# AutomationLabs-sh/AutomationLabsModelPredictiveControl.jl

Measured on AMD Instinct MI355X. Metric: MPC steps/s (batch=4096, nx=12, nu=4, N=30), higher is better.
Workload: dtype f64; 1 GPU; configs[1]: hover-linearised quadrotor nx=12 nu=4 N=30, 4096 instances per GPU, shared model, x0 amplitude classes 0.3/1.0/3.0 interleaved, cold start every step; batch_per_gpu=4096, global_batch=4096, seed=0x5eed0002, setup_ramp_steps=300, admm_max_iter=6, check_every=6, polish=1, warm_state_kept=False, parallelism=instances sharded over 1 GPU(s), 16-instance tile per workgroup

## Files before the change

automationlabsmodelpredictivecontrol.jl_amd/_capi.py:

```python
from __future__ import annotations

import ctypes
import os

import numpy as np

_HERE = os.path.dirname(os.path.abspath(__file__))
LIB_PATH = os.environ.get("ALMPC_LIB") or os.path.join(_HERE, "lib", "libalmpc.so")

ALMPC_OK = 0
ERR_NAMES = {0: "ALMPC_OK", -1: "ALMPC_ERR_INVALID", -2: "ALMPC_ERR_NO_DEVICE", -3: "ALMPC_ERR_HIP",
             -4: "ALMPC_ERR_UNSUPPORTED", -5: "ALMPC_ERR_NOT_DESIGNED", -6: "ALMPC_ERR_NUMERIC"}
FLAG_TIMING = 0x1
FLAG_STRUCTURED = 0x2
SOLVED, MAX_ITER, NON_FINITE, INFEASIBLE = 0, 1, 2, 3


class AlmpcError(RuntimeError):
    def __init__(self, code, msg=""):
        self.code = code
        super().__init__(f"{ERR_NAMES.get(code, code)}: {msg}")


class almpc_opts(ctypes.Structure):
# ... 144 lines not shown
    L.almpc_group_sqp_fnn_skipped.argtypes = [_hp, _ip]
    L.almpc_group_sqp_fnn_state_multipliers.argtypes = [_hp, _dp]
    L.almpc_group_sqp_fnn_solve.argtypes = [_hp, ctypes.c_int, ctypes.c_double, ctypes.POINTER(almpc_opts), _ip, _ip, _dp]
    L.almpc_group_x0_staging.argtypes = [_hp, ctypes.POINTER(_dp)]
    L.almpc_group_update_initialization_staged.argtypes = [_hp, ctypes.POINTER(_dp)]
    L.almpc_group_get_results_async.argtypes = [_hp, ctypes.c_uint32]
    L.almpc_group_get_results_wait.argtypes = [_hp, ctypes.c_int, _dp, _dp, _dp, _dp, _dp, _ip, _ip, _ip]
    for nm_ in ("almpc_group_set_terminal_equality", "almpc_group_set_rho_profile", "almpc_group_set_structured_fallback", "almpc_group_set_state_box",
                "almpc_group_design_batched", "almpc_group_relin_fnn_setup", "almpc_group_relin_fnn_step", "almpc_group_relin_fnn_step_async",
                "almpc_group_relin_fnn_advance", "almpc_group_advance_plant", "almpc_group_sqp_fnn_set_structured", "almpc_group_sqp_fnn_set_step_rule",
                "almpc_group_sqp_fnn_setup", "almpc_group_relin_densenet_setup", "almpc_group_sqp_densenet_setup", "almpc_group_sqp_fnn_start", "almpc_group_sqp_fnn_iterate", "almpc_group_sqp_fnn_skipped", "almpc_group_sqp_fnn_solve", "almpc_group_sqp_fnn_set_hessian",
                "almpc_group_sqp_fnn_set_row_multipliers", "almpc_group_sqp_fnn_state_multipliers",
                "almpc_group_x0_staging", "almpc_group_update_initialization_staged", "almpc_group_get_results_async", "almpc_group_get_results_wait"):
        getattr(L, nm_).restype = ctypes.c_int
    L.almpc_set_start_from.argtypes = [_hp, _hp]
    L.almpc_set_start_from.restype = ctypes.c_int
    L.almpc_timing_samples.argtypes = [_hp, ctypes.c_int, ctypes.POINTER(ctypes.c_int), _fp, _fp, _fp, _fp]
    L.almpc_timing_samples.restype = ctypes.c_int
    for name in ("almpc_x0_staging", "almpc_update_initialization_async", "almpc_get_results_async", "almpc_get_results_wait", "almpc_host_results",
                 "almpc_get_first_input", "almpc_group_create", "almpc_group_size", "almpc_group_shard", "almpc_group_design_shared",
                 "almpc_group_set_reference", "almpc_group_update_initialization", "almpc_group_calculate",
                 "almpc_group_calculate_async", "almpc_group_synchronize", "almpc_group_get_results"):
        getattr(L, name).restype = ctypes.c_int
    for name in ("almpc_create", "almpc_design_shared", "almpc_set_reference", "almpc_update_initialization",
                 "almpc_update_initialization_device", "almpc_calculate", "almpc_calculate_async", "almpc_synchronize",
                 "almpc_get_results", "almpc_get_design", "almpc_device_results", "almpc_get_timing", "almpc_timing_reset",
                 "almpc_timing_summary"):
        getattr(L, name).restype = ctypes.c_int
    _lib = L
    return L


OPT_NO_WARM_STATE = 0x1
WANT = {"x": 0x01, "e_x": 0x02, "u": 0x04, "e_u": 0x08, "status": 0x10, "iters": 0x20, "polish_iters": 0x40, "u0": 0x80}


def _want_mask(want):
    try:
        return sum(WANT[k] for k in set(want))
    except KeyError as e:
        raise ValueError(f"unknown result {e.args[0]!r}; choose from {sorted(WANT)}") from None


def comm_unique_id() -> bytes:
    buf = ctypes.create_string_buffer(128)
    rc = load().almpc_comm_unique_id(buf)
    if rc != ALMPC_OK:
        raise AlmpcError(rc, "almpc_comm_unique_id (librccl not loadable?)")
    return buf.raw


def default_opts(**kw) -> almpc_opts:
    o = almpc_opts()
    load().almpc_default_opts(ctypes.byref(o))
    if "keep_warm_state" in kw:
        if not kw.pop("keep_warm_state"):
            o.reserved[0] |= OPT_NO_WARM_STATE
    for k, v in kw.items():
        if not hasattr(o, k):
            raise TypeError(f"unknown solver option {k!r}")
        setattr(o, k, v)
    return o


def _colmajor(a, shape=None):
    a = np.asfortranarray(np.asarray(a, dtype=np.float64))
    if shape is not None and a.shape != shape:
        raise ValueError(f"expected shape {shape}, got {a.shape}")
    return a


def _ptr(a):
    return None if a is None else a.ctypes.data_as(_dp)


def dare(A, B, Q, R):
    L = load()
    A, B = np.asfortranarray(A, dtype=np.float64), np.asfortranarray(B, dtype=np.float64)
    n, m = B.shape
    Q, R = _colmajor(Q, (n, n)), _colmajor(R, (m, m))
    P = np.empty((n, n), order="F")
    rc = L.almpc_dare(n, m, _ptr(A), _ptr(B), _ptr(Q), _ptr(R), _ptr(P))
    if rc != ALMPC_OK:
        raise AlmpcError(rc, "almpc_dare")
    return P


FNN_ACTIVATIONS = {"identity": 0, "relu": 1, "tanh": 2, "sigmoid": 3, "swish": 4}
NET_KINDS = {"fnn", "resnet", "polynet"}
_NET_CODES = {"fnn": 0, "resnet": 1, "polynet": 2}
# ... 727 lines not shown
```

automationlabsmodelpredictivecontrol.jl_amd/csrc/almpc_api.hip:

```cpp
#include "almpc_kernels.hip.h"
#include "almpc_design.hip.h"
#include "almpc_polish_gen.hip.h"
#include "almpc_fnn.hip.h"
#include "almpc_instance.hip.h"
#include "almpc_sqp.hip.h"
#include "almpc_comm.hip.h"
#include "almpc_riccati.hip.h"
#include "almpc_sdual.hip.h"
#include "almpc_host_math.h"
#include "almpc_switches.h"
#include "../../include/almpc.h"

#ifndef ALMPC_UNITY
#define ALMPC_KERNEL_INSTANCE(...) extern template __global__ __VA_ARGS__;
#include "instances/sdual_a.inc"
#include "instances/sdual_b.inc"
#include "instances/sdual_c.inc"
#include "instances/polish_gen.inc"
#include "instances/step.inc"
#include "instances/instance.inc"
#include "instances/design_a.inc"
#include "instances/design_b.inc"
#undef ALMPC_KERNEL_INSTANCE
#endif
// ... 1948 lines not shown
    per_wave = (per_wave + 1) & ~1;
    if (h->batched) {
        L.wave_const_off = per_wave;
        per_wave += (h->nzs + h->n * (h->n + h->m) + 1) & ~1;
    }
    L.per_wave = per_wave;
    L.SL = polish_shared_layout(h->n, h->m, h->N, h->nz, h->nzs, L.fuse_rollout);
    L.g_lds = (size_t)h->nz * ((h->nz + 1) & ~1);
    L.l_glds = (L.g_lds + L.SL.total + (size_t)POLISH_WAVES_GLDS * per_wave + 2) * sizeof(double);
    const size_t slot = (size_t)POLISH_SG_SHARED_CAP * 64 * sizeof(double);
    if (L.l_glds + slot <= 160 * 1024 && !h->batched && !h->sw.polish_sg_global) {
        L.sg_shared_off = (int)(L.SL.total + (size_t)POLISH_WAVES_GLDS * per_wave + 2);
        L.l_glds += slot;
    }
    L.l_step = L.l_glds - L.g_lds * sizeof(double);
    if (admm_lds_bytes(h) > L.l_step) L.l_step = admm_lds_bytes(h);
    L.l_step += L.g_lds * sizeof(double);
    return L;
}

PolishParams polish_params(const Step& s, const PolishLayout& L) {
    const almpc_handle* h = s.h;
    PolishParams pp;
    pp.nz = h->nz; pp.m = h->m; pp.batch = h->batch; pp.nzs = h->nzs;
    pp.G = h->batched ? h->bG : h->dG; pp.dvec = h->batched ? h->bD : h->dD;
    pp.G_stride = h->batched ? (long)h->nz * h->nzs : 0; pp.d_stride = h->batched ? (long)h->nzs : 0;
    pp.A_stride = h->batched ? (long)h->n * h->n : 0; pp.B_stride = h->batched ? (long)h->n * h->m : 0;
    pp.wave_const_off = L.wave_const_off; pp.sg_off = 0; pp.g_off = 0; pp.sg_shared_off = L.sg_shared_off;
    pp.umin = h->dUmin; pp.umax = h->dUmax; pp.uref = h->dUref; pp.uref_stride = h->uref_stride;
    pp.zs = h->dZs; pp.ys = h->dYs; pp.v0 = h->dV0; pp.w = h->dW; pp.status = h->dStatus; pp.piters = h->dPiters;
    pp.yflags = s.keep_state ? nullptr : h->dYflags; pp.yflag_words = h->nrb;
    pp.sglobal = h->dSglobal; pp.perm = h->dPerm; pp.ntiles = (h->batch + 15) / 16;
    pp.max_iter = s.o.polish_max_iter > 0 ? s.o.polish_max_iter : 2 * h->nz + 50;
    pp.dflag = s.mode.fold_flag ? h->bFlag : nullptr;
    if (s.lazy_redo) { pp.unsolved = h->redo.dUnsolved; pp.redo_gate = h->redo.dGate; pp.step_serial = h->redo.step_serial; }
    pp.fuse_rollout = L.fuse_rollout; pp.roll_g = s.roll.g; pp.roll_cpl = s.roll.cpl; pp.roll = s.rp;
    pp.rollM = h->dRollM; pp.roll_s = h->roll_s; pp.roll_nb = h->roll_nb;
    pp.lds_per_wave = L.per_wave;
    return pp;
}

enum class Route { StateRows, FusedShared, WaveShared, WaveInst, TwoLaunch, NoPolish };

Route pick_route(const Step& s, const PolishLayout& L) {
    const almpc_handle* h = s.h;
    if (h->mc > 0) return Route::StateRows;
    if (!s.o.polish) return Route::NoPolish;
    if (!h->batched && h->fuse_step && POLISH_WAVES_GLDS == 8 && !h->sw.polish_no_glds && h->nrb == 8 && (h->ks == 30 || h->ks == 32) && L.fused &&
        L.l_step <= 160 * 1024)
        return Route::FusedShared;
    if (!h->batched && h->nzs <= 64 && L.fused && h->dPlain && !h->ltv && !h->sw.no_shared_wave &&
        (long)h->batch <= h->sw.shared_wave_max_batch.value_or((long)2 * h->num_cus) && ((size_t)L.SL.total + (size_t)L.per_wave) * sizeof(double) <= 64 * 1024)
        return Route::WaveShared;
    if (h->batched && s.mode.guess == Guess::Admm && h->nzs <= 64 && L.fused && !h->sw.no_inst_wave &&
        ((size_t)L.SL.total + (size_t)L.per_wave + (size_t)h->nz * h->nzs) * sizeof(double) <= 64 * 1024)
        return Route::WaveInst;
    return Route::TwoLaunch;
}

template <bool PACKED>
hipError_t launch_admm_inst(const AdmmInstParams& ip, int wgs, size_t lds, hipStream_t st) {
    if (lds > 64 * 1024) {
        const hipError_t e = ensure_dyn_lds(reinterpret_cast<const void*>(k_admm_inst<PACKED>), lds);
        if (e != hipSuccess) return e;
    }
    hipLaunchKernelGGL((k_admm_inst<PACKED>), dim3(wgs), dim3(ADMM_INST_THREADS), lds, st, ip);
// ... 1588 lines not shown
```

automationlabsmodelpredictivecontrol.jl_amd/csrc/almpc_kernels.hip.h:

```cpp
#pragma once
#include <hip/hip_runtime.h>
#include <stdint.h>

#include <map>
#include <mutex>
#include <utility>
#include <type_traits>

namespace almpc {

inline hipError_t ensure_dyn_lds(const void* fn, size_t bytes) {
    if (bytes <= 64 * 1024) return hipSuccess;
    static std::mutex mu;
    static std::map<std::pair<int, const void*>, size_t> cur;
    int dev = 0;
    hipError_t e = hipGetDevice(&dev);
    if (e != hipSuccess) return e;
    std::lock_guard<std::mutex> lock(mu);
    size_t& c = cur[std::make_pair(dev, fn)];
    if (c >= bytes) return hipSuccess;
    e = hipFuncSetAttribute(fn, hipFuncAttributeMaxDynamicSharedMemorySize, (int)bytes);
    if (e == hipSuccess) c = bytes;
    return e;
}


#ifdef ALMPC_STAMPS
__device__ long long* g_stamps = nullptr;
#define ALMPC_STAMP(WAVE_ID, SLOT)                                                                     \
    do {                                                                                               \
        __builtin_amdgcn_sched_barrier(0);                                                             \
        if (g_stamps && (threadIdx.x & 63) == 0) g_stamps[(size_t)(WAVE_ID) * 16 + (SLOT)] = __builtin_readcyclecounter(); \
        __builtin_amdgcn_sched_barrier(0);                                                             \
    } while (0)
#define ALMPC_ACC_DECL long long acc_t[8] = {0, 0, 0, 0, 0, 0, 0, 0}; long long acc_prev = 0; int acc_n = 0;
#define ALMPC_ACC_START do { __builtin_amdgcn_sched_barrier(0); acc_prev = __builtin_readcyclecounter(); __builtin_amdgcn_sched_barrier(0); } while (0)
#define ALMPC_ACC(SLOT) do { __builtin_amdgcn_sched_barrier(0); const long long n_ = __builtin_readcyclecounter(); acc_t[SLOT] += n_ - acc_prev; acc_prev = n_; __builtin_amdgcn_sched_barrier(0); } while (0)
#define ALMPC_ACC_FLUSH(WAVE_ID) do { if (g_stamps && (threadIdx.x & 63) == 0) { for (int i_ = 0; i_ < 8; ++i_) g_stamps[(size_t)(4096 + (WAVE_ID)) * 16 + i_] = acc_t[i_]; g_stamps[(size_t)(4096 + (WAVE_ID)) * 16 + 8] = acc_n; } } while (0)
#else
#define ALMPC_STAMP(WAVE_ID, SLOT) do { } while (0)
#define ALMPC_ACC_DECL
#define ALMPC_ACC_START do { } while (0)
#define ALMPC_ACC(SLOT) do { } while (0)
#define ALMPC_ACC_FLUSH(WAVE_ID) do { } while (0)
#endif

__host__ __device__ inline int packed_tri_off(int nz, int c) {
    const int full = c * nz - (c * (c - 1)) / 2;
    const int pads = (nz & 1) ? (c / 2) : ((c + 1) / 2);
    return full + pads;
}
__host__ __device__ inline long packed_tri_doubles(int nz) { return ((long)packed_tri_off(nz, nz) + 1) & ~1L; }

typedef double d4 __attribute__((ext_vector_type(4)));
typedef double d2v __attribute__((ext_vector_type(2)));

constexpr int TILE = 16;

__device__ __forceinline__ d4 mfma_f64(double a, double b, d4 c) {
    return __builtin_amdgcn_mfma_f64_16x16x4f64(a, b, c, 0, 0, 0);
}

template <int KS>
__device__ __forceinline__ d4 tile_matmul(const double (&a)[KS], const double* bbuf, int q, int col) {
    d4 acc0 = {0.0, 0.0, 0.0, 0.0}, acc1 = {0.0, 0.0, 0.0, 0.0};
#pragma unroll
    for (int ks = 0; ks < KS; ks += 2) {
        double b0 = bbuf[(4 * ks + q) * TILE + col];
        acc0 = mfma_f64(a[ks], b0, acc0);
        if (ks + 1 < KS) {
            double b1 = bbuf[(4 * (ks + 1) + q) * TILE + col];
// ... 212 lines not shown
        if (check) {
            double rp = 0, nx = 0, nzn = 0, rd = 0, nhx = 0, ny = 0, bad = 0;
            for (int w2 = 0; w2 < NRB; ++w2) {
                const double* r = red + w2 * 8 * TILE + col;
                rp = fmax(rp, r[0 * TILE]); nx = fmax(nx, r[1 * TILE]); nzn = fmax(nzn, r[2 * TILE]);
                rd = fmax(rd, r[3 * TILE]); nhx = fmax(nhx, r[4 * TILE]); ny = fmax(ny, r[5 * TILE]);
                bad = fmax(bad, r[6 * TILE]);
            }
            if (active) {
                const bool conv = (rp <= p.eps_abs + p.eps_rel * fmax(nx, nzn)) &&
                                  (rd <= p.eps_abs + p.eps_rel * fmax(fmax(nhx, ny), nf));
                if (bad > 0.0) { active = false; my_iters = it; my_status = 2; }
                else if (conv) { active = false; my_iters = it; my_status = 0; }
            }
            const bool any_active = __any(active);
            __syncthreads();
            if (!any_active) { double* t = cur; cur = nxt; nxt = t; break; }
        }
        double* t = cur; cur = nxt; nxt = t;
    }

    ALMPC_STAMP(blockIdx.x * NRB + wv, 2);
#pragma unroll
    for (int ks = 0; ks < KSF_MAX; ++ks)
        af[ks] = (ks < p.ksf) ? p.VFrag[((size_t)(wv * p.ksf + ks)) * 64 + lane] : 0.0;
    double v0s[4];
#pragma unroll
    for (int i = 0; i < 4; ++i) v0s[i] = (row[i] < p.nz) ? p.v0S[(size_t)instc * p.v0S_stride + row[i]] : 0.0;
    if (valid && wv == 0 && q == 0) {
        p.iters[inst] = my_iters;
        p.status[inst] = my_status;
        p.piters[inst] = 0;
    }
    {
        int cntf = 0;
#pragma unroll
        for (int i = 0; i < 4; ++i) cntf += (row[i] < p.nz && yt[i] != 0.0) ? 1 : 0;
        cntf += __shfl_xor(cntf, 16);
        cntf += __shfl_xor(cntf, 32);
        if (q == 0) red[(wv * 8 + 0) * TILE + col] = (double)cntf;
    }
    __syncthreads();
    if (wv == 0 && q == 0) {
        int k0 = valid ? 0 : -1;
        if (valid)
            for (int w2 = 0; w2 < NRB; ++w2) k0 += (int)red[(w2 * 8 + 0) * TILE + col];
        red[(0 * 8 + 1) * TILE + col] = (double)k0;
        __builtin_amdgcn_fence(__ATOMIC_RELEASE, "wavefront");
        __builtin_amdgcn_wave_barrier();
        __builtin_amdgcn_fence(__ATOMIC_ACQUIRE, "wavefront");
        int rank = 0;
        for (int c2 = 0; c2 < TILE; ++c2) {
            const int ko = (int)red[(0 * 8 + 1) * TILE + c2];
            rank += (ko > k0 || (ko == k0 && c2 < col)) ? 1 : 0;
        }
        p.perm[blockIdx.x * TILE + rank] = valid ? inst : -1;
    }
    d4 v04 = {v0s[0], v0s[1], v0s[2], v0s[3]};
#pragma unroll
    for (int ks = 0; ks < KSF_MAX; ++ks)
        if (ks < p.ksf) v04 = mfma_f64(af[ks], e0s[(4 * ks + q) * TILE + col], v04);
    ALMPC_STAMP(blockIdx.x * NRB + wv, 3);

    constexpr int TS = RP + 2;
    static_assert(TILE * TS <= 2 * RP * TILE, "staging tile must fit the two rhs buffers");
    double* stage = smem;
    auto flush = [&](const double (&v)[4], double* dst) {
        __syncthreads();
#pragma unroll
        for (int i = 0; i < 4; ++i) stage[col * TS + row[i]] = v[i];
        __syncthreads();
        for (int e = 2 * threadIdx.x; e < TILE * RP; e += 2 * blockDim.x) {
            const int ci = e / RP, r = e % RP;
            const int ii = blockIdx.x * TILE + ci;
            if (ii < p.batch)
                *reinterpret_cast<d2v*>(dst + (size_t)ii * p.nzs + r) = *reinterpret_cast<const d2v*>(stage + ci * TS + r);
        }
    };
    const double v0r[4] = {v04[0], v04[1], v04[2], v04[3]};
    double y[4];
#pragma unroll
    for (int i = 0; i < 4; ++i) y[i] = rho[i] * yt[i];
    if (p.keep_state) {
        flush(x, p.xs);
        flush(y, p.ys);
    } else {
        uint32_t mk = 0;
#pragma unroll
        for (int i = 0; i < 4; ++i) {
            const uint32_t b = (uint32_t)(q + 4 * i);
            mk |= (yt[i] < 0.0 ? 1u : 0u) << b;
            mk |= (yt[i] > 0.0 ? 1u : 0u) << (16u + b);
        }
        mk |= (uint32_t)__shfl_xor((int)mk, 16);
// ... 28 lines not shown
    double* x;
    double* ex;
    double* u;
    double* eu;
};

struct PolishParams {
    int nz, m, batch, nzs;
    const double* G;
    const double* dvec;
    const double* umin;
    const double* umax;
    const double* uref;
    long uref_stride;
    const double* zs;
    const double* ys;
    const uint32_t* yflags;
    int yflag_words;
    const double* v0;
    double* w;
    int32_t* status;
    int32_t* piters;
    double* sglobal;
    const int32_t* start_rows = nullptr;
    const int32_t* perm;
    int ntiles;
    int lds_per_wave;
    long G_stride, d_stride, A_stride, B_stride;
    int wave_const_off;
    int sg_off;
    int sg_shared_off;
    int g_off;
    int max_iter;
    const int* dflag = nullptr;
    int* unsolved = nullptr;
    int* redo_gate = nullptr;
    int step_serial = 0;
    int direct = 0;
    int fuse_rollout;
    int roll_g, roll_cpl;
    const double* rollM;
    int roll_s, roll_nb;
    RolloutParams roll;
};

__device__ __forceinline__ double readlane_d(double v, int l) {
    int lo = __builtin_amdgcn_readlane(__double2loint(v), l);
    int hi = __builtin_amdgcn_readlane(__double2hiint(v), l);
    return __hiloint2double(hi, lo);
}

__device__ __forceinline__ double fast_rcp_d(double v) {
    double r = __builtin_amdgcn_rcp(v);
    r = __builtin_fma(__builtin_fma(-v, r, 1.0), r, r);
    r = __builtin_fma(__builtin_fma(-v, r, 1.0), r, r);
    return r;
}

typedef double gj16_row[16];
template <int JJ>
__device__ __forceinline__ void gj16_pivot(gj16_row& r, const double (&pj)[16], const double col, const double d, const bool own, const int k,
                                           const int lane) {
    const double invd = fast_rcp_d(d);
    const bool piv = lane == k;
    const double f = piv ? -invd : col * invd;
    const double keep = piv ? 0.0 : 1.0;
// ... 195 lines not shown
    }
}

constexpr int POLISH_WAVES = 4;
#ifndef ALMPC_EXP_POLISH_WAVES
#define ALMPC_EXP_POLISH_WAVES 8
#endif
constexpr int POLISH_WAVES_GLDS = ALMPC_EXP_POLISH_WAVES;
constexpr int POLISH_LDS_MIN_PER_WAVE = 128 + 64 + 64 + 32;
struct PolishShared {
    int off_d, off_umin, off_umax, off_uref, off_ab, off_xref, total;
};
__host__ __device__ inline PolishShared polish_shared_layout(int n, int m, int N, int nz, int nzs, int fused) {
    PolishShared L;
    L.off_d = 0;
    L.off_umin = nzs;
    L.off_umax = L.off_umin + m;
    L.off_uref = L.off_umax + m;
    L.off_ab = L.off_uref + nz;
    L.off_xref = L.off_ab + ((fused && fused != 3) ? n * (n + m) : 0);
    L.total = (L.off_xref + (fused ? (N + 1) * n : 0) + 1) & ~1;
    return L;
}
constexpr int POLISH_GLB_PER_INST = 64 * 64;
constexpr int POLISH_SG_SHARED_CAP = 48;

typedef double d2 __attribute__((ext_vector_type(2)));

template <bool GLDS, bool GPRE, int KOFF, bool SGL = false, bool START = false>
__device__ __forceinline__ void polish_body(const PolishParams& p_arg, double* smem) {
    const PolishParams& p = p_arg;
    constexpr int CH = (GLDS || SGL) ? 8 : 16;
    constexpr int NWV = GLDS ? POLISH_WAVES_GLDS : (SGL ? 1 : POLISH_WAVES);
    const int wv = __builtin_amdgcn_readfirstlane(threadIdx.x >> 6), lane_k = threadIdx.x & 63;
    const int nz = p.nz, nzs = p.nzs;
    const double* Gp = p.G;
    const int gs = GLDS ? ((nz + 1) & ~1) : nzs;
    const PolishShared SL = polish_shared_layout(p.roll.n, p.m, p.roll.N, nz, nzs, p.fuse_rollout);
    double* shc = smem + (GLDS ? (size_t)nz * gs : 0);
    double* wave_lds = shc + SL.total + (size_t)wv * p.lds_per_wave;
    int* qcnt = nullptr;
    const bool uref_sh = p.uref_stride == 0, xref_sh = p.roll.xref_stride == 0;
    const bool per_inst = p.G_stride != 0;
    double* cd = shc + SL.off_d;
    double* cab = shc + SL.off_ab;
    if (per_inst) { cd = wave_lds + p.wave_const_off; cab = cd + nzs; }
    {
        constexpr int TPB = 64 * NWV;
        const int n = p.roll.n, m = p.m, N = p.roll.N;
        if (!per_inst)
            for (int t = threadIdx.x; t < nzs; t += TPB) shc[SL.off_d + t] = p.dvec[t];
        for (int t = threadIdx.x; t < m; t += TPB) { shc[SL.off_umin + t] = p.umin[t]; shc[SL.off_umax + t] = p.umax[t]; }
        if (uref_sh)
            for (int t = threadIdx.x; t < nz; t += TPB) shc[SL.off_uref + t] = p.uref[t];
        if (p.fuse_rollout) {
            if (!per_inst && p.fuse_rollout != 3) {
                for (int t = threadIdx.x; t < n * n; t += TPB) shc[SL.off_ab + t] = p.roll.A[t];
                for (int t = threadIdx.x; t < n * m; t += TPB) shc[SL.off_ab + n * n + t] = p.roll.B[t];
            }
            if (xref_sh)
                for (int t = threadIdx.x; t < (N + 1) * n; t += TPB) shc[SL.off_xref + t] = p.roll.xref[t];
        }
    }
    ALMPC_STAMP(8192 + blockIdx.x * 8 + wv, 0);
    if constexpr (GLDS && !GPRE) {
        const int hs = gs / 2;
// ... 85 lines not shown
        const d2 zz = *reinterpret_cast<const d2*>(GL(p.zs) + base + rc);
        v00 = vv[0]; v01 = vv[1]; y0 = yy[0]; y1 = yy[1]; z0 = zz[0]; z1 = zz[1];
        double urp0, urp1;
        if (uref_sh) {
            urp0 = shc[SL.off_uref + (in0 ? r0 : 0)]; urp1 = shc[SL.off_uref + (in1 ? r1 : 0)];
            asm volatile("" : "+v"(urp0), "+v"(urp1));
        } else {
            const double* ug = GL(p.uref) + (size_t)inst * p.uref_stride;
            urp0 = ug[in0 ? r0 : 0]; urp1 = ug[in1 ? r1 : 0];
        }
        if (in0) {
            const double di = 1.0 / dv[0], ur = urp0;
            lo0 = (shc[SL.off_umin + r0 % p.m] - ur) * di; hi0 = (shc[SL.off_umax + r0 % p.m] - ur) * di; w0 = fmin(fmax(z0, lo0), hi0);
        } else { v00 = 0.0; y0 = 0.0; z0 = 0.0; }
        if (in1) {
            const double di = 1.0 / dv[1], ur = urp1;
            lo1 = (shc[SL.off_umin + r1 % p.m] - ur) * di; hi1 = (shc[SL.off_umax + r1 % p.m] - ur) * di; w1 = fmin(fmax(z1, lo1), hi1);
        } else { v01 = 0.0; y1 = 0.0; z1 = 0.0; }
    }
    int wrow = 0, wsd = 0;
    double wbnd = 0.0;
    double lam = 0.0;
    bool act0 = false, act1 = false;
    double bnd0 = 0.0, bnd1 = 0.0;
    double t0 = v00, t1 = v01;
    int k = 0;
    bool overflow = false;
    ALMPC_ACC_DECL
    wrow_s[lane] = 0;
    const int hpos = lane & 31, hhf = lane >> 5;
    double Sr[16];
#pragma unroll
    for (int t = 0; t < 16; ++t) Sr[t] = 0.0;
    auto bcast16 = [&](const double* buf, double (&o)[16]) {
#pragma unroll
        for (int t = 0; t < 8; ++t) {
            const d2 v = *reinterpret_cast<const d2*>(buf + 16 * hhf + 2 * t);
            o[2 * t] = v[0]; o[2 * t + 1] = v[1];
        }
    };
    auto col_to_buf = [&](int j, double* buf) {
        const int tj = j & 15;
        double v = Sr[0];
#pragma unroll
        for (int t = 1; t < 16; ++t) {
            double x = Sr[t];
            asm volatile("" : "+v"(x));
            v = (tj == t) ? x : v;
        }
        if (hhf == (j >> 4)) buf[hpos] = v;
        wave_fence_lds();
    };
    ALMPC_STAMP(inst, 9);

    auto sync_s = [&](auto m) {
        if (decltype(m)::glb && !sg_lds) {
            __builtin_amdgcn_fence(__ATOMIC_RELEASE, "workgroup");
            __builtin_amdgcn_wave_barrier();
            __builtin_amdgcn_fence(__ATOMIC_ACQUIRE, "workgroup");
        } else {
            wave_fence_lds();
        }
    };
    auto sptr = [&](auto) -> double* { return Sg; };
    auto put_pos = [&](auto m, double* buf, double v) {
        buf[decltype(m)::half ? (lane & 31) : lane] = v;
// ... 11 lines not shown
            for (int t = 0; t < 16; t += 2) { acc += Sr[t] * cv[t]; acc2 += Sr[t + 1] * cv[t + 1]; }
            acc = half_sum(acc + acc2);
        } else {
            double* S = sptr(m);
            for (int l0 = 0; l0 < k; l0 += 8) {
                double sv[8], cv[8];
#pragma unroll
                for (int t = 0; t < 8; ++t) { sv[t] = S[(l0 + t) * M::WL + lane]; cv[t] = cb[l0 + t]; }
#pragma unroll
                for (int t = 0; t < 8; ++t) acc += sv[t] * cv[t];
            }
        }
        return acc;
    };
    auto s_rank1 = [&](auto m, double a, const double* ab, double scale) {
        using M = decltype(m);
        const double as = a * scale;
        if constexpr (M::half) {
            double av[16];
            bcast16(ab, av);
#pragma unroll
            for (int t = 0; t < 16; ++t) Sr[t] = __builtin_fma(as, av[t], Sr[t]);
        } else {
            double* S = sptr(m);
            for (int l0 = 0; l0 < k; l0 += 8) {
                double cur[8], av[8];
#pragma unroll
                for (int t = 0; t < 8; ++t) { cur[t] = S[(l0 + t) * M::WL + lane]; av[t] = ab[l0 + t]; }
#pragma unroll
                for (int t = 0; t < 8; ++t) S[(l0 + t) * M::WL + lane] = cur[t] + as * av[t];
            }
        }
    };
    auto g_load = [&](int l0, d2 (&g)[CH]) {
#ifdef ALMPC_EXP_ROWS_READLANE
#pragma unroll
        for (int t = 0; t < CH; ++t) g[t] = *reinterpret_cast<const d2*>(Gp + (__builtin_amdgcn_readlane(wrow, l0 + t) * gs + rc));
#else
        typedef int i4 __attribute__((ext_vector_type(4)));
        int rows[CH];
#pragma unroll
        for (int t = 0; t < CH; t += 4) {
            const i4 r4 = *reinterpret_cast<const i4*>(wrow_s + l0 + t);
            rows[t] = r4[0]; rows[t + 1] = r4[1]; rows[t + 2] = r4[2]; rows[t + 3] = r4[3];
        }
#pragma unroll
        for (int t = 0; t < CH; ++t) g[t] = *reinterpret_cast<const d2*>(Gp + (rows[t] * gs + rc));
#endif
    };
    auto g_fma = [&](int l0, const double* ab, const d2 (&g)[CH], double& q0, double& q1) {
        double av[CH];
#pragma unroll
        for (int t = 0; t < CH; ++t) av[t] = ab[l0 + t];
#pragma unroll
        for (int t = 0; t < CH; ++t) { q0 += g[t][0] * av[t]; q1 += g[t][1] * av[t]; }
    };
    auto g_rows_times = [&](const double* ab, double& q0, double& q1) {
        q0 = 0.0; q1 = 0.0;
        for (int l0 = 0; l0 < k; l0 += CH) {
            d2 g[CH];
            g_load(l0, g);
            g_fma(l0, ab, g, q0, q1);
        }
    };
    auto put_rows = [&](double a0, double a1) {
        d2 v; v[0] = a0; v[1] = a1;
        *reinterpret_cast<d2*>(rowbuf + r0) = v;
        wave_fence_lds();
    };
    auto recompute = [&](auto m) {
        using M = decltype(m);
        const int pos = M::half ? (lane & 31) : lane;
        put_rows(v00, v01);
        const double rv = rowbuf[wrow] - wbnd;
        put_pos(m, pbufa, (pos < k) ? rv : 0.0);
        const double lm = s_matvec(m, pbufa);
        lam = (pos < k) ? lm : 0.0;
        put_pos(m, pbufb, lam);
        double q0, q1;
        g_rows_times(pbufb, q0, q1);
        t0 = v00 - q0;
        t1 = v01 - q1;
    };
    auto add_row = [&](auto m, int j, double bval, int sd) {
        using M = decltype(m);
        const int pos = M::half ? (lane & 31) : lane;
        const bool lowhalf = M::half ? (lane < 32) : true;
        ALMPC_ACC_START;
        const d2 gj = *reinterpret_cast<const d2*>(Gp + (j * gs + rc));
        d2 g[CH];
        g_load(0, g);
        const double cv = Gp[j * gs + wrow];
        const double gjj = Gp[j * gs + j];
        const double c = (pos < k) ? cv : 0.0;
        const double tj = readlane_d((j & 1) ? t1 : t0, j >> 1);
        ALMPC_ACC(0);
        put_pos(m, pbufa, c);
        const double u = s_matvec(m, pbufa);
        ALMPC_ACC(1);
        put_pos(m, pbufb, u);
        double q0 = 0.0, q1 = 0.0;
        g_fma(0, pbufb, g, q0, q1);
        for (int l0 = CH; l0 < k; l0 += CH) {
            g_load(l0, g);
            g_fma(l0, pbufb, g, q0, q1);
        }
        ALMPC_ACC(2);
        const double sc = gjj - wave_sum(lowhalf ? c * u : 0.0);
        const double isc = fast_rcp_d(sc);
        const double mu = (tj - bval) * isc;
        t0 -= mu * (gj[0] - q0);
        t1 -= mu * (gj[1] - q1);
        lam -= u * mu;
        ALMPC_ACC(3);
        if constexpr (M::half) {
            if (lane == k) {
                double m1 = -1.0;
                asm volatile("" : "+v"(m1));
                pbufb[hpos] = m1;
            }
            wave_fence_lds();
            double av[16];
            bcast16(pbufb, av);
            const double as = (pos == k) ? -isc : u * isc;
#pragma unroll
            for (int t = 0; t < 16; ++t) Sr[t] = __builtin_fma(as, av[t], Sr[t]);
        } else {
            double* S = sptr(m);
            s_rank1(m, u, pbufb, isc);
            const double bv = (pos == k) ? isc : -u * isc;
            S[k * M::WL + pos] = bv;
            if (pos < cap2) S[pos * M::WL + k] = bv;
        }
        if (pos == k) { wrow = j; wsd = sd; wbnd = bval; lam = mu; }
        if (lane == 0) wrow_s[k] = j;
        if (r0 == j) { act0 = true; bnd0 = bval; }
        if (r1 == j) { act1 = true; bnd1 = bval; }
        k += 1;
        sync_s(m);
        ALMPC_ACC(4);
#ifdef ALMPC_STAMPS
        acc_n += 1;
#endif
    };
    auto remove_pos = [&](auto m, int rp) {
        using M = decltype(m);
        const int pos = M::half ? (lane & 31) : lane;
        const int last = k - 1;
        const int jrem = __builtin_amdgcn_readlane(wrow, rp);
        if constexpr (M::half) {
            col_to_buf(rp, pbufb);
            const double sp = pbufb[pos];
            double av[16];
            bcast16(pbufb, av);
            const double spp = readlane_d(sp, rp);
            const double a = readlane_d(lam, rp) / spp;
            double q0, q1;
            g_rows_times(pbufb, q0, q1);
            t0 += a * q0;
            t1 += a * q1;
            lam -= sp * a;
            const double as = -sp / spp;
#pragma unroll
            for (int t = 0; t < 16; ++t) Sr[t] = __builtin_fma(as, av[t], Sr[t]);
            if (rp != last) {
                col_to_buf(last, pbufa);
                const double colv = pbufa[pos];
                const double corner = readlane_d(colv, last);
                const double nv = (pos == rp) ? corner : ((pos == last) ? 0.0 : colv);
                put_pos(m, pbufa, nv);
                double rv[16];
                bcast16(pbufa, rv);
#pragma unroll
                for (int t = 0; t < 16; ++t) Sr[t] = (pos == rp) ? rv[t] : ((16 * hhf + t == rp) ? nv : Sr[t]);
                const int lrow = __builtin_amdgcn_readlane(wrow, last), lsd = __builtin_amdgcn_readlane(wsd, last);
                const double lbv = readlane_d(wbnd, last), llam = readlane_d(lam, last);
                if (pos == rp) { wrow = lrow; wsd = lsd; wbnd = lbv; lam = llam; }
                if (lane == 0) wrow_s[rp] = lrow;
            }
#pragma unroll
            for (int t = 0; t < 16; ++t) Sr[t] = (pos == last || 16 * hhf + t == last) ? 0.0 : Sr[t];
        } else {
// ... 18 lines not shown
                const int lrow = __builtin_amdgcn_readlane(wrow, last), lsd = __builtin_amdgcn_readlane(wsd, last);
                const double lbv = readlane_d(wbnd, last), llam = readlane_d(lam, last);
                if (pos == rp) { wrow = lrow; wsd = lsd; wbnd = lbv; lam = llam; }
                if (lane == 0) wrow_s[rp] = lrow;
            }
            {
                const double iv = (pos == last) ? 1.0 : 0.0;
                S[last * M::WL + pos] = iv;
                if (pos < cap2) S[pos * M::WL + last] = iv;
            }
        }
        if (pos == last) lam = 0.0;
        if (lane == 0) wrow_s[last] = 0;
        if (r0 == jrem) act0 = false;
        if (r1 == jrem) act1 = false;
        k -= 1;
        sync_s(m);
    };

    int it = 0;
    int fin = 1;
    bool fresh = true;
    const int max_iter = p.max_iter;
    auto run = [&](auto m) {
        using M = decltype(m);
        const int pos = M::half ? (lane & 31) : lane;
        const bool lowhalf = M::half ? (lane < 32) : true;
        while (it < max_iter) {
            ++it;
            ALMPC_ACC_START;
            double rr = __builtin_inf();
            int rside = 0;
            bool second = false;
            {
                const bool f0 = in0 && !act0, f1 = in1 && !act1;
                const bool up0 = t0 > hi0, dn0 = t0 < lo0, up1 = t1 > hi1, dn1 = t1 < lo1;
                const double c0 = ((up0 ? hi0 : lo0) - w0) * fast_rcp_d(t0 - w0);
                const double c1 = ((up1 ? hi1 : lo1) - w1) * fast_rcp_d(t1 - w1);
                const bool v0 = f0 && (up0 || dn0), v1 = f1 && (up1 || dn1);
                if (v0) { rr = c0; rside = up0 ? 1 : -1; }
                if (v1 && (!v0 || c1 < c0)) { rr = c1; rside = up1 ? 1 : -1; second = true; }
            }
            const double rmin = wave_min(rr);
            if (rmin < 1.0) {
                if (k == (M::glb ? cap2 : M::WL)) { --it; overflow = true; return; }
                const int owner = __builtin_ctzll(__ballot(rr == rmin));
                const double bcand = second ? (rside > 0 ? hi1 : lo1) : (rside > 0 ? hi0 : lo0);
                const int jmin = 2 * owner + (__builtin_amdgcn_readlane(second ? 1 : 0, owner));
                const int sd = __builtin_amdgcn_readlane(rside, owner);
                const double bval = readlane_d(bcand, owner);
                const double tt = fmax(rmin, 0.0);
                if (in0 && !act0) w0 += tt * (t0 - w0);
                if (in1 && !act1) w1 += tt * (t1 - w1);
                if (r0 == jmin) w0 = bval;
                if (r1 == jmin) w1 = bval;
                ALMPC_ACC(5);
                add_row(m, jmin, bval, sd);
                fresh = false;
                continue;
            }
            if (!act0) w0 = t0;
            if (!act1) w1 = t1;
            bool ok = true;
            int vi = 0;
            if (k > 0) {
                const bool mine = lowhalf && pos < k;
                const double viol = mine ? ((wsd > 0) ? -lam : lam) : -__builtin_inf();
                const double lmax = wave_max(mine ? fabs(lam) : 0.0);
                const double vmax = wave_max(viol);
                ok = vmax <= 1e-12 * fmax(1.0, lmax);
                vi = __builtin_ctzll(__ballot(mine && viol == vmax));
            }
            if (ok) {
                if (fresh) { fin = 0; return; }
                recompute(m);
                fresh = true;
                --it;
                continue;
            }
            remove_pos(m, vi);
            fresh = false;
        }
    };
    auto tier2_home = [&](int need) {
        if constexpr (GLDS) {
            if (p.sg_shared_off >= 0 && need <= POLISH_SG_SHARED_CAP) {
                int got = 0;
                if (lane == 0) got = (atomicCAS(qcnt + 1, -1, wv) == -1) ? 1 : 0;
                got = __builtin_amdgcn_readfirstlane(got);
                if (got) { own_slot = true; cap2 = POLISH_SG_SHARED_CAP; Sg = shc + p.sg_shared_off; }
// ... 342 lines not shown
#pragma unroll
            for (int u = 0; u < 4; ++u) {
                const int t = t0 + 64 * u + lane;
                if (t < nx) {
                    GL(rp.ex)[xo + t] = ev[u];
                    GL(rp.x)[xo + t] = (t < n) ? x0r : ev[u] + xr[u];
                }
            }
        }
        ALMPC_STAMP(inst, 14);
    }
  };

    if constexpr (GLDS) {
        ALMPC_STAMP(8192 + blockIdx.x * 8 + wv, 1);
        [[maybe_unused]] int nproc = 0;
        for (int i = wv;;) {
            const int tile = (i >> 4) * (int)gridDim.x + (int)blockIdx.x;
            if (tile >= p.ntiles) break;
            const int inst = p.perm[tile * 16 + (i & 15)];
            if (inst >= 0) {
                process(inst);
                ++nproc;
            }
            if (lane_k == 0) i = atomicAdd(qcnt, 1);
            i = __builtin_amdgcn_readfirstlane(i);
        }
        ALMPC_STAMP(8192 + blockIdx.x * 8 + wv, 2);
#ifdef ALMPC_STAMPS
        if (g_stamps && (threadIdx.x & 63) == 0) g_stamps[(size_t)(8192 + blockIdx.x * 8 + wv) * 16 + 3] = nproc;
#endif
    } else {
        const int slot = blockIdx.x * NWV + wv;
        if (p.direct) {
            if (slot < p.batch) process(slot);
        } else if (slot < p.ntiles * 16) {
            const int inst = p.perm[(slot % p.ntiles) * 16 + slot / p.ntiles];
            if (inst >= 0) process(inst);
        }
    }
}

template <bool GLDS>
__global__ __launch_bounds__(64 * (GLDS ? POLISH_WAVES_GLDS : POLISH_WAVES))
__attribute__((amdgpu_waves_per_eu(GLDS ? POLISH_WAVES_GLDS / 4 : 2, GLDS ? POLISH_WAVES_GLDS / 4 : 2)))
void k_polish(PolishParams p_arg) {
    extern __shared__ __attribute__((aligned(16))) double smem[];
    polish_body<GLDS, false, 0>(p_arg, smem);
}

template <int START = 0>
__global__ __launch_bounds__(64) void k_polish_sgl(PolishParams p_arg) {
    extern __shared__ __attribute__((aligned(16))) double smem[];
    polish_body<false, false, 0, true, START != 0>(p_arg, smem);
}

constexpr int STEP_KOFF = (int)((sizeof(AdmmParams) + 7) & ~size_t(7));

template <int NRB, int KS>
__global__ __launch_bounds__(64 * NRB) __attribute__((amdgpu_waves_per_eu(2, 2)))
void k_step_fused(AdmmParams ap, PolishParams pp) {
    extern __shared__ __attribute__((aligned(16))) double smem[];
    if constexpr (NRB != POLISH_WAVES_GLDS) return;
    const int wv = __builtin_amdgcn_readfirstlane(threadIdx.x >> 6), lane = threadIdx.x & 63;
    const int gs = (pp.nz + 1) & ~1, hs = gs / 2;
    auto request_g = [&]() __attribute__((always_inline)) {
        for (int r = wv; r < pp.nz; r += NRB) {
            if (lane < hs) {
                const char* src = reinterpret_cast<const char*>(pp.G + (size_t)r * pp.nzs) + lane * 16;
                __builtin_amdgcn_global_load_lds((const __attribute__((address_space(1))) void*)src,
                                                 (__attribute__((address_space(3))) void*)(smem + (size_t)r * gs), 16, 0, 0);
            }
// ... 106 lines not shown
```

include/almpc.h:

```cpp
#ifndef ALMPC_H
#define ALMPC_H

#include <stdint.h>

#ifdef __cplusplus
extern "C" {
#endif

#define ALMPC_VERSION_MAJOR 0
#define ALMPC_VERSION_MINOR 1

typedef struct almpc_handle almpc_handle;

typedef enum almpc_status {
    ALMPC_OK = 0,
    ALMPC_ERR_INVALID = -1,
    ALMPC_ERR_NO_DEVICE = -2,
    ALMPC_ERR_HIP = -3,
    ALMPC_ERR_UNSUPPORTED = -4,
    ALMPC_ERR_NOT_DESIGNED = -5,
    ALMPC_ERR_NUMERIC = -6
} almpc_status;

typedef enum almpc_solve_status {
    ALMPC_SOLVED = 0,
    ALMPC_MAX_ITER = 1,
    ALMPC_NON_FINITE = 2,
    ALMPC_INFEASIBLE = 3
} almpc_solve_status;

typedef struct almpc_opts {
    double rho;
    double sigma;
    double alpha;
    double eps_abs;
    double eps_rel;
    int32_t max_iter;
    int32_t check_every;
    int32_t polish;
    int32_t polish_max_iter;
    int32_t warm_start;
    int32_t reserved[3];
} almpc_opts;

#define ALMPC_OPT_NO_WARM_STATE 0x1

void almpc_default_opts(almpc_opts* opts);

#define ALMPC_FLAG_TIMING 0x1u
#define ALMPC_FLAG_STRUCTURED 0x2u

int almpc_create(almpc_handle** out, int n, int m, int N, int batch, int device_id, uint32_t flags);
void almpc_destroy(almpc_handle* h);
const char* almpc_last_error(const almpc_handle* h);

int almpc_set_terminal_equality(almpc_handle* h, int on);

int almpc_set_rho_profile(almpc_handle* h, int mode);

int almpc_set_step_fusion(almpc_handle* h, int on);

int almpc_set_structured_fallback(almpc_handle* h, int on);

int almpc_set_start_from(almpc_handle* h, almpc_handle* src);

int almpc_set_state_box(almpc_handle* h, const double* xmin, const double* xmax);

int almpc_design_shared(almpc_handle* h, const double* A, const double* B, const double* Q,
                        const double* R, const double* S, const double* P, const double* umin,
                        const double* umax, const double* xmin, const double* xmax, double rho,
                        double sigma);

int almpc_design_batched(almpc_handle* h, const double* A_batch, const double* B_batch, const double* Q,
                         const double* R, const double* S, const double* P, int P_per_instance,
                         const double* umin, const double* umax, double rho, double sigma);

int almpc_design_ltv(almpc_handle* h, const double* A_all, const double* B_all, const double* c_all, const double* xbar,
                     const double* ubar, const double* xref, const double* uref, const double* Q, const double* R,
// ... 174 lines not shown
```

Baseline: 16860 batch-steps/s (one step = 4096 instance QP solves).

## Add lookahead precomputation of likely next active-set rows in polish solver

In the active-set polish, when a row is added to the factorization, the kernel now also speculatively computes projected columns and Schur updates for up to two candidate rows expected to enter next: the paired slack row and the runner-up blocking constraint. If the next added row matches a cached candidate, the expensive G row gather and matvec are skipped. The cached candidates are kept current through rank-one updates on each later addition. The tile sort key also now counts initially violated bounds, weighted heavily, so instances with similar expected work are grouped together. The trade-off is extra FMA work and register pressure on every miss.

```diff
diff --git a/automationlabsmodelpredictivecontrol.jl_amd/_capi.py b/automationlabsmodelpredictivecontrol.jl_amd/_capi.py
--- a/automationlabsmodelpredictivecontrol.jl_amd/_capi.py
+++ b/automationlabsmodelpredictivecontrol.jl_amd/_capi.py
@@ -200,6 +200,7 @@
 
 
 OPT_NO_WARM_STATE = 0x1
+OPT_NO_LOOKAHEAD = 0x2
 WANT = {"x": 0x01, "e_x": 0x02, "u": 0x04, "e_u": 0x08, "status": 0x10, "iters": 0x20, "polish_iters": 0x40, "u0": 0x80}
 
 
@@ -224,6 +225,9 @@
     if "keep_warm_state" in kw:
         if not kw.pop("keep_warm_state"):
             o.reserved[0] |= OPT_NO_WARM_STATE
+    if "lookahead" in kw:
+        if not kw.pop("lookahead"):
+            o.reserved[0] |= OPT_NO_LOOKAHEAD
     for k, v in kw.items():
         if not hasattr(o, k):
             raise TypeError(f"unknown solver option {k!r}")
diff --git a/automationlabsmodelpredictivecontrol.jl_amd/csrc/almpc_api.hip b/automationlabsmodelpredictivecontrol.jl_amd/csrc/almpc_api.hip
--- a/automationlabsmodelpredictivecontrol.jl_amd/csrc/almpc_api.hip
+++ b/automationlabsmodelpredictivecontrol.jl_amd/csrc/almpc_api.hip
@@ -2004,6 +2004,7 @@
     pp.yflags = s.keep_state ? nullptr : h->dYflags; pp.yflag_words = h->nrb;
     pp.sglobal = h->dSglobal; pp.perm = h->dPerm; pp.ntiles = (h->batch + 15) / 16;
     pp.max_iter = s.o.polish_max_iter > 0 ? s.o.polish_max_iter : 2 * h->nz + 50;
+    pp.lookahead = (s.o.reserved[0] & ALMPC_OPT_NO_LOOKAHEAD) ? 0 : 1;
     pp.dflag = s.mode.fold_flag ? h->bFlag : nullptr;
     if (s.lazy_redo) { pp.unsolved = h->redo.dUnsolved; pp.redo_gate = h->redo.dGate; pp.step_serial = h->redo.step_serial; }
     pp.fuse_rollout = L.fuse_rollout; pp.roll_g = s.roll.g; pp.roll_cpl = s.roll.cpl; pp.roll = s.rp;
diff --git a/automationlabsmodelpredictivecontrol.jl_amd/csrc/almpc_kernels.hip.h b/automationlabsmodelpredictivecontrol.jl_amd/csrc/almpc_kernels.hip.h
--- a/automationlabsmodelpredictivecontrol.jl_amd/csrc/almpc_kernels.hip.h
+++ b/automationlabsmodelpredictivecontrol.jl_amd/csrc/almpc_kernels.hip.h
@@ -33,10 +33,10 @@
         if (g_stamps && (threadIdx.x & 63) == 0) g_stamps[(size_t)(WAVE_ID) * 16 + (SLOT)] = __builtin_readcyclecounter(); \
         __builtin_amdgcn_sched_barrier(0);                                                             \
     } while (0)
-#define ALMPC_ACC_DECL long long acc_t[8] = {0, 0, 0, 0, 0, 0, 0, 0}; long long acc_prev = 0; int acc_n = 0;
+#define ALMPC_ACC_DECL long long acc_t[8] = {0, 0, 0, 0, 0, 0, 0, 0}; long long acc_prev = 0; int acc_n = 0, acc_h = 0;
 #define ALMPC_ACC_START do { __builtin_amdgcn_sched_barrier(0); acc_prev = __builtin_readcyclecounter(); __builtin_amdgcn_sched_barrier(0); } while (0)
 #define ALMPC_ACC(SLOT) do { __builtin_amdgcn_sched_barrier(0); const long long n_ = __builtin_readcyclecounter(); acc_t[SLOT] += n_ - acc_prev; acc_prev = n_; __builtin_amdgcn_sched_barrier(0); } while (0)
-#define ALMPC_ACC_FLUSH(WAVE_ID) do { if (g_stamps && (threadIdx.x & 63) == 0) { for (int i_ = 0; i_ < 8; ++i_) g_stamps[(size_t)(4096 + (WAVE_ID)) * 16 + i_] = acc_t[i_]; g_stamps[(size_t)(4096 + (WAVE_ID)) * 16 + 8] = acc_n; } } while (0)
+#define ALMPC_ACC_FLUSH(WAVE_ID) do { if (g_stamps && (threadIdx.x & 63) == 0) { for (int i_ = 0; i_ < 8; ++i_) g_stamps[(size_t)(4096 + (WAVE_ID)) * 16 + i_] = acc_t[i_]; g_stamps[(size_t)(4096 + (WAVE_ID)) * 16 + 8] = acc_n; g_stamps[(size_t)(4096 + (WAVE_ID)) * 16 + 9] = acc_h; } } while (0)
 #else
 #define ALMPC_STAMP(WAVE_ID, SLOT) do { } while (0)
 #define ALMPC_ACC_DECL
@@ -315,10 +315,20 @@
         p.status[inst] = my_status;
         p.piters[inst] = 0;
     }
+    d4 v04 = {v0s[0], v0s[1], v0s[2], v0s[3]};
+#pragma unroll
+    for (int ks = 0; ks < KSF_MAX; ++ks)
+        if (ks < p.ksf) v04 = mfma_f64(af[ks], e0s[(4 * ks + q) * TILE + col], v04);
+    constexpr int KEY_GUESS = 1024;
+    static_assert(RP <= KEY_GUESS, "the tie-breaker must not carry into the key");
     {
         int cntf = 0;
 #pragma unroll
-        for (int i = 0; i < 4; ++i) cntf += (row[i] < p.nz && yt[i] != 0.0) ? 1 : 0;
+        for (int i = 0; i < 4; ++i) {
+            const bool in = row[i] < p.nz;
+            cntf += (in && yt[i] != 0.0) ? 1 : 0;
+            cntf += (in && (v04[i] < lo[i] || v04[i] > hi[i])) ? KEY_GUESS : 0;
+        }
         cntf += __shfl_xor(cntf, 16);
         cntf += __shfl_xor(cntf, 32);
         if (q == 0) red[(wv * 8 + 0) * TILE + col] = (double)cntf;
@@ -339,10 +349,6 @@
         }
         p.perm[blockIdx.x * TILE + rank] = valid ? inst : -1;
     }
-    d4 v04 = {v0s[0], v0s[1], v0s[2], v0s[3]};
-#pragma unroll
-    for (int ks = 0; ks < KSF_MAX; ++ks)
-        if (ks < p.ksf) v04 = mfma_f64(af[ks], e0s[(4 * ks + q) * TILE + col], v04);
     ALMPC_STAMP(blockIdx.x * NRB + wv, 3);
 
     constexpr int TS = RP + 2;
@@ -437,6 +443,7 @@
     int sg_shared_off;
     int g_off;
     int max_iter;
+    int lookahead = 1;
     const int* dflag = nullptr;
     int* unsolved = nullptr;
     int* redo_gate = nullptr;
@@ -698,6 +705,8 @@
     const PolishParams& p = p_arg;
     constexpr int CH = (GLDS || SGL) ? 8 : 16;
     constexpr int NWV = GLDS ? POLISH_WAVES_GLDS : (SGL ? 1 : POLISH_WAVES);
+    constexpr bool LA = !SGL;
+    constexpr int LA_MIN_ROWS = 16;
     const int wv = __builtin_amdgcn_readfirstlane(threadIdx.x >> 6), lane_k = threadIdx.x & 63;
     const int nz = p.nz, nzs = p.nzs;
     const double* Gp = p.G;
@@ -849,6 +858,9 @@
     double Sr[16];
 #pragma unroll
     for (int t = 0; t < 16; ++t) Sr[t] = 0.0;
+    [[maybe_unused]] int la_row[2] = {-1, -1};
+    [[maybe_unused]] double la_p0[2] = {0.0, 0.0}, la_p1[2] = {0.0, 0.0}, la_u[2] = {0.0, 0.0};
+    [[maybe_unused]] const bool la_on = LA && p.lookahead != 0;
     auto bcast16 = [&](const double* buf, double (&o)[16]) {
 #pragma unroll
         for (int t = 0; t < 8; ++t) {
@@ -926,20 +938,21 @@
             }
         }
     };
-    auto g_load = [&](int l0, d2 (&g)[CH]) {
+    auto g_load = [&](int l0, auto& g) {
+        constexpr int CL = (int)(sizeof(g) / sizeof(d2));
 #ifdef ALMPC_EXP_ROWS_READLANE
 #pragma unroll
-        for (int t = 0; t < CH; ++t) g[t] = *reinterpret_cast<const d2*>(Gp + (__builtin_amdgcn_readlane(wrow, l0 + t) * gs + rc));
+        for (int t = 0; t < CL; ++t) g[t] = *reinterpret_cast<const d2*>(Gp + (__builtin_amdgcn_readlane(wrow, l0 + t) * gs + rc));
 #else
         typedef int i4 __attribute__((ext_vector_type(4)));
-        int rows[CH];
-#pragma unroll
-        for (int t = 0; t < CH; t += 4) {
+        int rows[CL];
+#pragma unroll
+        for (int t = 0; t < CL; t += 4) {
             const i4 r4 = *reinterpret_cast<const i4*>(wrow_s + l0 + t);
             rows[t] = r4[0]; rows[t + 1] = r4[1]; rows[t + 2] = r4[2]; rows[t + 3] = r4[3];
         }
 #pragma unroll
-        for (int t = 0; t < CH; ++t) g[t] = *reinterpret_cast<const d2*>(Gp + (rows[t] * gs + rc));
+        for (int t = 0; t < CL; ++t) g[t] = *reinterpret_cast<const d2*>(Gp + (rows[t] * gs + rc));
 #endif
     };
     auto g_fma = [&](int l0, const double* ab, const d2 (&g)[CH], double& q0, double& q1) {
@@ -976,11 +989,75 @@
         t0 = v00 - q0;
         t1 = v01 - q1;
     };
-    auto add_row = [&](auto m, int j, double bval, int sd) {
+    auto add_row = [&](auto m, int j, double bval, int sd, int hit = -1, int ca0 = -1, int ca1 = -1) {
         using M = decltype(m);
+        constexpr bool la_m = LA && M::half;
         const int pos = M::half ? (lane & 31) : lane;
         const bool lowhalf = M::half ? (lane < 32) : true;
         ALMPC_ACC_START;
+        double u, pj0, pj1, isc, mu;
+        if (la_m && hit >= 0) {
+            u = hit == 0 ? la_u[0] : la_u[1];
+            pj0 = hit == 0 ? la_p0[0] : la_p0[1];
+            pj1 = hit == 0 ? la_p1[0] : la_p1[1];
+            if (hit == 0) la_row[0] = -1; else la_row[1] = -1;
+            const double sc = readlane_d((j & 1) ? pj1 : pj0, j >> 1);
+            const double tj = readlane_d((j & 1) ? t1 : t0, j >> 1);
+            isc = fast_rcp_d(sc);
+            mu = (tj - bval) * isc;
+            put_pos(m, pbufb, u);
+            ALMPC_ACC(6);
+#ifdef ALMPC_STAMPS
+            acc_h += 1;
+#endif
+        } else if (la_m && (ca0 >= 0 || ca1 >= 0)) {
+            const int a0 = ca0 >= 0 ? ca0 : 0, a1 = ca1 >= 0 ? ca1 : 0;
+            double* lc0 = pbufa + 32; double* lu0 = pbufb + 32; double* lc1 = rowbuf; double* lu1 = rowbuf + 32;
+            const d2 gj = *reinterpret_cast<const d2*>(Gp + (j * gs + rc));
+            constexpr int CL = 8;
+            d2 g[CL];
+            g_load(0, g);
+            const double cv = Gp[j * gs + wrow];
+            const double gjj = Gp[j * gs + j];
+            const double cva0 = Gp[a0 * gs + wrow], cva1 = Gp[a1 * gs + wrow];
+            const d2 ga0 = *reinterpret_cast<const d2*>(Gp + (a0 * gs + rc)), ga1 = *reinterpret_cast<const d2*>(Gp + (a1 * gs + rc));
+            const double c = (pos < k) ? cv : 0.0;
+            const double tj = readlane_d((j & 1) ? t1 : t0, j >> 1);
+            ALMPC_ACC(0);
+            lc0[hpos] = (pos < k) ? cva0 : 0.0;
+            lc1[hpos] = (pos < k) ? cva1 : 0.0;
+            put_pos(m, pbufa, c);
+            u = s_matvec(m, pbufa);
+            const double ua0 = s_matvec(m, lc0), ua1 = s_matvec(m, lc1);
+            ALMPC_ACC(1);
+            lu0[hpos] = ua0;
+            lu1[hpos] = ua1;
+            put_pos(m, pbufb, u);
+            double q0 = 0.0, q1 = 0.0, pa00 = ga0[0], pa01 = ga0[1], pa10 = ga1[0], pa11 = ga1[1];
+            for (int l0 = 0; l0 < k; l0 += CL) {
+                if (l0 > 0) g_load(l0, g);
+#pragma unroll
+                for (int t4 = 0; t4 < CL; t4 += 4) {
+                    double av[4], av0[4], av1[4];
+#pragma unroll
+                    for (int t = 0; t < 4; ++t) { av[t] = pbufb[l0 + t4 + t]; av0[t] = lu0[l0 + t4 + t]; av1[t] = lu1[l0 + t4 + t]; }
+#pragma unroll
+                    for (int t = 0; t < 4; ++t) {
+                        q0 += g[t4 + t][0] * av[t]; q1 += g[t4 + t][1] * av[t];
+                        pa00 = __builtin_fma(-g[t4 + t][0], av0[t], pa00); pa01 = __builtin_fma(-g[t4 + t][1], av0[t], pa01);
+                        pa10 = __builtin_fma(-g[t4 + t][0], av1[t], pa10); pa11 = __builtin_fma(-g[t4 + t][1], av1[t], pa11);
+                    }
+                }
+            }
+            ALMPC_ACC(2);
+            const double sc = gjj - wave_sum(lowhalf ? c * u : 0.0);
+            isc = fast_rcp_d(sc);
+            mu = (tj - bval) * isc;
+            pj0 = gj[0] - q0;
+            pj1 = gj[1] - q1;
+            if (ca0 >= 0) { la_row[0] = ca0; la_p0[0] = pa00; la_p1[0] = pa01; la_u[0] = ua0; }
+            if (ca1 >= 0) { la_row[1] = ca1; la_p0[1] = pa10; la_p1[1] = pa11; la_u[1] = ua1; }
+        } else {
         const d2 gj = *reinterpret_cast<const d2*>(Gp + (j * gs + rc));
         d2 g[CH];
         g_load(0, g);
@@ -990,7 +1067,7 @@
         const double tj = readlane_d((j & 1) ? t1 : t0, j >> 1);
         ALMPC_ACC(0);
         put_pos(m, pbufa, c);
-        const double u = s_matvec(m, pbufa);
+        u = s_matvec(m, pbufa);
         ALMPC_ACC(1);
         put_pos(m, pbufb, u);
         double q0 = 0.0, q1 = 0.0;
@@ -1001,11 +1078,26 @@
         }
         ALMPC_ACC(2);
         const double sc = gjj - wave_sum(lowhalf ? c * u : 0.0);
-        const double isc = fast_rcp_d(sc);
-        const double mu = (tj - bval) * isc;
-        t0 -= mu * (gj[0] - q0);
-        t1 -= mu * (gj[1] - q1);
+        isc = fast_rcp_d(sc);
+        mu = (tj - bval) * isc;
+        pj0 = gj[0] - q0;
+        pj1 = gj[1] - q1;
+        }
+        t0 -= mu * pj0;
+        t1 -= mu * pj1;
         lam -= u * mu;
+        if constexpr (la_m) {
+#pragma unroll
+            for (int s = 0; s < 2; ++s) {
+                const int a = la_row[s];
+                if (a >= 0) {
+                    const double f = readlane_d((a & 1) ? pj1 : pj0, a >> 1) * isc;
+                    la_p0[s] = __builtin_fma(-pj0, f, la_p0[s]);
+                    la_p1[s] = __builtin_fma(-pj1, f, la_p1[s]);
+                    la_u[s] = (pos == k) ? f : __builtin_fma(-u, f, la_u[s]);
+                }
+            }
+        }
         ALMPC_ACC(3);
         if constexpr (M::half) {
             if (lane == k) {
@@ -1042,6 +1134,7 @@
         const int pos = M::half ? (lane & 31) : lane;
         const int last = k - 1;
         const int jrem = __builtin_amdgcn_readlane(wrow, rp);
+        la_row[0] = -1; la_row[1] = -1;
         if constexpr (M::half) {
             col_to_buf(rp, pbufb);
             const double sp = pbufb[pos];
@@ -1126,15 +1219,13 @@
             double rr = __builtin_inf();
             int rside = 0;
             bool second = false;
-            {
-                const bool f0 = in0 && !act0, f1 = in1 && !act1;
-                const bool up0 = t0 > hi0, dn0 = t0 < lo0, up1 = t1 > hi1, dn1 = t1 < lo1;
-                const double c0 = ((up0 ? hi0 : lo0) - w0) * fast_rcp_d(t0 - w0);
-                const double c1 = ((up1 ? hi1 : lo1) - w1) * fast_rcp_d(t1 - w1);
-                const bool v0 = f0 && (up0 || dn0), v1 = f1 && (up1 || dn1);
-                if (v0) { rr = c0; rside = up0 ? 1 : -1; }
-                if (v1 && (!v0 || c1 < c0)) { rr = c1; rside = up1 ? 1 : -1; second = true; }
-            }
+            const bool f0 = in0 && !act0, f1 = in1 && !act1;
+            const bool up0 = t0 > hi0, dn0 = t0 < lo0, up1 = t1 > hi1, dn1 = t1 < lo1;
+            const double c0 = ((up0 ? hi0 : lo0) - w0) * fast_rcp_d(t0 - w0);
+            const double c1 = ((up1 ? hi1 : lo1) - w1) * fast_rcp_d(t1 - w1);
+            const bool v0 = f0 && (up0 || dn0), v1 = f1 && (up1 || dn1);
+            if (v0) { rr = c0; rside = up0 ? 1 : -1; }
+            if (v1 && (!v0 || c1 < c0)) { rr = c1; rside = up1 ? 1 : -1; second = true; }
             const double rmin = wave_min(rr);
             if (rmin < 1.0) {
                 if (k == (M::glb ? cap2 : M::WL)) { --it; overflow = true; return; }
@@ -1143,13 +1234,34 @@
                 const int jmin = 2 * owner + (__builtin_amdgcn_readlane(second ? 1 : 0, owner));
                 const int sd = __builtin_amdgcn_readlane(rside, owner);
                 const double bval = readlane_d(bcand, owner);
+                int hit = -1, ca0 = -1, ca1 = -1;
+                if constexpr (LA && M::half) {
+                    if (la_on) {
+                        hit = (jmin == la_row[0]) ? 0 : ((jmin == la_row[1]) ? 1 : -1);
+                        if (hit < 0 && k >= LA_MIN_ROWS) {
+                            const int js = jmin + p.m;
+                            if (js < nz && ((__builtin_amdgcn_readlane((f0 ? 1 : 0) | (f1 ? 2 : 0), js >> 1) >> (js & 1)) & 1) != 0) ca0 = js;
+                            const bool own = lane == owner;
+                            const bool sec2 = own ? !second : second;
+                            const double rr2 = own ? (second ? (v0 ? c0 : __builtin_inf()) : (v1 ? c1 : __builtin_inf())) : rr;
+                            const double rmin2 = wave_min(rr2);
+                            if (rmin2 < __builtin_inf()) {
+                                const int owner2 = __builtin_ctzll(__ballot(rr2 == rmin2));
+                                ca1 = 2 * owner2 + (__builtin_amdgcn_readlane(sec2 ? 1 : 0, owner2));
+                            }
+                            if (ca1 == ca0) ca1 = -1;
+                            if (ca0 >= 0 && ca1 < 0 && la_row[1] == ca0) la_row[1] = -1;
+                            if (ca1 >= 0 && ca0 < 0 && la_row[0] == ca1) la_row[0] = -1;
+                        }
+                    }
+                }
                 const double tt = fmax(rmin, 0.0);
                 if (in0 && !act0) w0 += tt * (t0 - w0);
                 if (in1 && !act1) w1 += tt * (t1 - w1);
                 if (r0 == jmin) w0 = bval;
                 if (r1 == jmin) w1 = bval;
                 ALMPC_ACC(5);
-                add_row(m, jmin, bval, sd);
+                add_row(m, jmin, bval, sd, hit, ca0, ca1);
                 fresh = false;
                 continue;
             }
@@ -1558,12 +1670,13 @@
 #endif
     } else {
         const int slot = blockIdx.x * NWV + wv;
+        int inst = -1;
         if (p.direct) {
-            if (slot < p.batch) process(slot);
+            if (slot < p.batch) inst = slot;
         } else if (slot < p.ntiles * 16) {
-            const int inst = p.perm[(slot % p.ntiles) * 16 + slot / p.ntiles];
-            if (inst >= 0) process(inst);
-        }
+            inst = p.perm[(slot % p.ntiles) * 16 + slot / p.ntiles];
+        }
+        if (inst >= 0) process(inst);
     }
 }
 
diff --git a/include/almpc.h b/include/almpc.h
--- a/include/almpc.h
+++ b/include/almpc.h
@@ -44,6 +44,7 @@
 } almpc_opts;
 
 #define ALMPC_OPT_NO_WARM_STATE 0x1
+#define ALMPC_OPT_NO_LOOKAHEAD 0x2
 
 void almpc_default_opts(almpc_opts* opts);
 
```

Result: slower. 15580 batch-steps/s (one step = 4096 instance QP solves) (-7.6%).
